# bioinformatics-centre/BayesTyper

Hardware: AMD Instinct MI355X
Metric: variant-cluster Gibbs iterations/sec + k-mer matches/sec at 1/2/4/8 MI355X (higher is better)
Workload: dtype f64 log-probabilities over u8 k-mer counts (Gibbs); u64/u8 integer (k-mer matching)

## Files before the change

bayestyper_amd/csrc/bt_gibbs_kernel.hpp:

```cpp
#pragma once
#include "bt_gibbs_tile.hpp"
#include "bt_noise_chain.hpp"
#include "bt_noise_help.hpp"
#include "bt_gibbs_simple.hpp"

namespace bt {

enum GibbsOp { OP_RUN = 0, OP_INIT_CHAIN = 1, OP_SWEEP = 2, OP_NOISE = 3, OP_RESET = 4, OP_SETUP = 5, OP_NOISE_CHAIN = 6 };

struct TraceCfg {
    uint32_t max_sweeps;
    uint32_t *counter;
    uint32_t *buf;
};

__device__ BT_NOINLINE void group_init_chain(Env env, uint32_t chain, uint32_t nvert, uint32_t nsrc, uint32_t gindex) {
    const Tile t = make_tile(env);
    const GParams BT_CAS &P = env_params(env);
    const uint32_t gseed = P.noise_seeding ? P.seed + (gindex + 1u) * (chain + 1u) : P.seed + (gindex + 1u);
    for (uint32_t v = 0; v < nvert; ++v) {
        const Vx c = make_vx(t, v);
        Env ev = env;
        const bool swap = env.resident == 0xFFFFFFFFu && t.d->hot_bytes != 0;
        if (swap) {
            hot_swap(env, v, true);
            ev.resident = v;
        }
        PROF_DECL;
        if (!make_vx(make_tile(ev), v).sc()[SC_CONSTRUCTED]) genotyper_construct(ev, v, gseed + c.cid());
        genotyper_reset(ev, v);
        if (swap) hot_swap(env, v, false);
    }
    if (nvert == 1 && nsrc == 1) return;
    uint32_t *bst = (uint32_t *)(t.base + t.d->off[A_BRNG]) + (size_t)t.plane * MT_PAD;
    mt_seed(bst, P.seed + (gindex + 1u) * (chain + 1u));
    Mt brng = mt_open(bst);
    rng_shuffle_u32(brng, t.arr<uint32_t>(A_SOURCES), nsrc);
    for (uint32_t v = 0; v < nvert; ++v) {
        const Vx c = make_vx(t, v);
        rng_shuffle_u32(brng, c.edges(), vx_ne(c));
    }
}

__device__ BT_NOINLINE void prepare_nested(Env env, uint32_t v_parent, uint32_t v_child) {
    if (env.resident != RESIDENT_ALL && env.resident != RESIDENT_NEVER) env.resident = 0xFFFFFFFFu;
    const Tile t = make_tile(env);
    const GParams BT_CAS &P = env_params(env);
    const Vx c = make_vx(t, v_parent), cc = make_vx(t, v_child);
    const uint32_t nd_n = vx_nd(c), cc_cid = cc.cid();
    const TileDesc BT_CAS &d = c.d();
    TPtr<uint32_t> ndcl = c.a<uint32_t>(A_NDCL, d.NDm > 1 ? d.NDm : 1), ndvo = c.a<uint32_t>(A_NDVOFF, d.NDm + 1);
    TPtr<uint16_t> ndv = c.a<uint16_t>(A_NDVAR, d.NDVm > 1 ? d.NDVm : 1);
    TPtr<uint32_t> pver = c.nver(), cver = cc.nver();
    for (uint32_t s = 0; s < P.S; ++s) {
        const uint32_t pv = pver[s];
        if (cver[P.S + s] == pv) continue;
        cver[P.S + s] = pv;
        cver[s] += 1;
        uint8_t ploidy = c.nest_ploidy()[s];
        uint32_t n = c.nest_n()[s];
        for (uint32_t j = 0; j < n; ++j)
            for (int q = 0; q < 4; ++q) cc.nest_stats(s, j)[q] = (double)c.nest_stats(s, j)[q];
        for (uint32_t which = 0; which < 2; ++which) {
            const uint16_t h = c.dip()[2 * s + which];
            if (h == NOHAP) continue;
            bool found = false;
            uint32_t lo = c.hn_off(h), hi = c.hn_off(h + 1);
            while (lo < hi) {
                const uint32_t mid = (lo + hi) >> 1;
                const uint32_t val = c.hn_idx(mid);
                if (val == cc_cid) {
                    found = true;
                    break;
                }
                if (val < cc_cid) lo = mid + 1;
                else hi = mid;
            }
            if (found) continue;
            ploidy = ploidy == 2 ? 1 : 0;
            uint32_t variant_idx = 0xFFFFFFFFu;
            for (uint32_t dd = 0; dd < nd_n; ++dd) {
                if (ndcl[dd] != cc_cid) continue;
                for (uint32_t i = ndvo[dd], i1 = ndvo[dd + 1]; i < i1; ++i) {
                    const uint32_t nv = ndv[i];
                    const uint32_t a = c.hap_allele(h, nv);
                    if (!is_missing(c, nv, a)) {
                        variant_idx = nv;
                        break;
                    }
                }
                break;
            }
            if (variant_idx != 0xFFFFFFFFu && n < 2) {
                for (int q = 0; q < 4; ++q) cc.nest_stats(s, n)[q] = (double)c.ksc(s, which, variant_idx)[q];
                ++n;
            }
        }
        cc.nest_ploidy()[s] = ploidy;
        cc.nest_n()[s] = (uint8_t)n;
    }
}

__device__ __forceinline__ void visit_vertex(const Env &env_in, const Tile &t, const GParams BT_CAS &P, uint32_t v, bool collect, TPtr<uint32_t> trace_row, bool tracing) {
    Env env = env_in;
    const bool swap = env.resident == 0xFFFFFFFFu && t.d->hot_bytes != 0;
    PROF_DECL;
    if (swap) {
        hot_swap(env, v, true);
        env.resident = v;
    }
    PROF(13);
    rng_topup(env, v);
    PROF(11);
    sample_diplotypes(env, v, collect, trace_row.off + v * P.S * LANES, tracing, (uint32_t *)trace_row.base);
    sample_haplotype_frequencies(env, v);
    PROF_DECL2;
    if (swap) hot_swap(env, v, false);
    PROF(13);
}

__device__ __forceinline__ void group_sweep(const Env &env, const Tile &t, const GParams BT_CAS &P, bool collect, uint32_t nvert, uint32_t nsrc, TPtr<uint32_t> trace_row, bool tracing) {
    if (tracing)
        for (uint32_t i = 0; i < t.d->nvm * P.S; ++i) trace_row[i] = 0xFFFFFFFFu;
    TPtr<uint32_t> sources = t.arr<uint32_t>(A_SOURCES), stack = t.arr<uint32_t>(A_STACK);
    TPtr<uint8_t> gploidy = t.arr<uint8_t>(A_PLOIDY);
    for (uint32_t si = 0; si < nsrc; ++si) {
        const uint32_t sv = sources[si];
        {
            const Vx root = make_vx(t, sv);
            for (uint32_t s = 0; s < P.S; ++s) {
                root.nest_ploidy()[s] = gploidy[s];
                root.nest_n()[s] = 0;
            }
        }
        uint32_t next = sv, sp = 0;
        bool have = true;
        while (have) {
            visit_vertex(env, t, P, next, collect, trace_row, tracing);
            if (nvert == 1) break;
            stack[2 * sp] = next;
            stack[2 * sp + 1] = 0;
            ++sp;
            have = false;
            while (sp > 0 && !have) {
                const uint32_t v = stack[2 * (sp - 1)];
                const uint32_t i = stack[2 * (sp - 1) + 1];
                const Vx c = make_vx(t, v);
                if (i < vx_ne(c)) {
                    stack[2 * (sp - 1) + 1] = i + 1;
                    const uint32_t tv = c.edges()[i];
                    {
                        PROF_DECL;
                        prepare_nested(env, v, tv);
                        PROF(14);
                    }
                    next = tv;
                    have = true;
                } else
                    --sp;
            }
        }
    }
}

__device__ BT_NOINLINE void noise_tally_group(Env env, uint32_t nvert, const NoiseChainCtl *nc) {
    if (env.resident != RESIDENT_ALL && env.resident != RESIDENT_NEVER) env.resident = 0xFFFFFFFFu;
    const Tile t = make_tile(env);
    const GParams BT_CAS &P = env_params(env);
    auto *bins = nc_bins(nc);
    for (uint32_t v = 0; v < nvert; ++v) {
        const Vx c = make_vx(t, v);
        const uint32_t nsu = c.sc()[SC_NSUB_U], Hm = t.d->Hm;
        const Vx::RPtr<uint8_t> sm = c.subm();
        TPtr<uint8_t> scn = c.subcnt(), sic = c.subic();
        for (uint32_t s = 0; s < P.S; ++s) {
            const uint16_t h1 = c.dip()[2 * s], h2 = c.dip()[2 * s + 1];
            const uint8_t gender = P.gender[s];
            for (uint32_t i = t.part; i < nsu; i += t.copies) {
                uint8_t m = sic[2 * i + gender];
                if (h1 != NOHAP) m = (uint8_t)(m + sm[i * Hm + h1]);
                if (h2 != NOHAP) m = (uint8_t)(m + sm[i * Hm + h2]);
                if (m == 0) nc_tally(nc, bins, s, scn[i * P.S + s]);
            }
        }
        if (t.part == 0) cache_clear(c, P, false, false);
        if (nc->help_units && help_table(t.d->cache_mode, t.d->simple, t.d->cache_entries, t.d->hoff[A_UCACHE], t.d->Dcm)) {
            if (t.copies > 1u) copies_sync();
            noise_help_publish(t, c);
        }
    }
    if (t.copies > 1u) copies_sync();
    if (nc->help_units && help_table(t.d->cache_mode, t.d->simple, t.d->cache_entries, t.d->hoff[A_UCACHE], t.d->Dcm)) __builtin_amdgcn_fence(__ATOMIC_RELEASE, "agent");
}

struct TraceRow {
    TPtr<uint32_t> row;
    bool on;
};
__device__ inline TraceRow trace_row_for(const Tile &t, const GParams BT_CAS &P, const TraceCfg &tr, uint32_t tile) {
    TraceRow r{TPtr<uint32_t>{(uint32_t BT_GAS *)tr.buf, 0u, 6u}, false};
    if (!tr.max_sweeps) return r;
    uint32_t *cnt = &tr.counter[(size_t)tile * LANES + t.lane];
    const uint32_t n = *cnt;
    if (n >= tr.max_sweeps) return r;
    *cnt = n + 1;
    r.row = TPtr<uint32_t>{(uint32_t BT_GAS *)tr.buf, (uint32_t)(t.d->trace_base + (size_t)n * t.d->nvm * P.S * LANES) + t.lane, 6u};
    r.on = true;
    return r;
}

#ifndef GIBBS_WAVES
#define GIBBS_WAVES 1
#endif
template <bool SIMPLE_ONLY>
__device__ __forceinline__ void gibbs_body(const TileDesc *__restrict__ tiles, uint8_t *__restrict__ pool, const GParams *__restrict__ Pg, int op, uint32_t arg0, uint32_t arg1,
                                           unsigned long long *__restrict__ hist, TraceCfg tr, const uint32_t *__restrict__ tile_list) {
    const uint32_t tile = kPacked ? ((const uint32_t BT_CAS *)tile_list)[2u * pack_slot()] : (tile_list ? tile_list[blockIdx.x] : blockIdx.x);
    if (kPacked && tile == 0xFFFFFFFFu) return;
    Env env{tiles, pool, Pg, tile_list, 0xFFFFFFFFu};
    const GParams BT_CAS &P = *(const GParams BT_CAS *)Pg;
    Tile t;
    t.d = (const TileDesc BT_CAS *)&tiles[tile];
    t.base = (uint8_t BT_GAS *)(pool + t.d->base);
    if (!tile_thread_active(tile_split(t.d), t.d->copies)) return;
    t.lane = tile_lane(tile_split(t.d), t.d->copies);
    t.plane = t.lane + t.d->pool_lane0;
    t.wsh = t.d->wsh;
    t.part = tile_part(t.d->copies);
    t.copies = t.d->copies;
    if (t.part != 0 && !(op == OP_RUN || op == OP_SWEEP || op == OP_INIT_CHAIN || op == OP_NOISE || op == OP_NOISE_CHAIN)) return;
    t.hot = nullptr;
    t.lds0 = kPacked ? ((const uint32_t BT_CAS *)tile_list)[2u * pack_slot() + 1u] : 0u;
    t.resident = 0xFFFFFFFFu;
    if (t.d->prio) __builtin_amdgcn_s_setprio(3);
    TPtr<uint32_t> gd = t.arr<uint32_t>(A_GDIMS);
    if (!gd[3]) return;
    const uint32_t nvert = kSingle ? 1u : (uint32_t)gd[0], nsrc = kSingle ? 1u : (uint32_t)gd[1], gindex = gd[2];
#ifdef BT_NO_NOISE_CHAIN
    const bool is_nc = false;
#else
    const bool is_nc = op == OP_NOISE_CHAIN;
#endif
    const NoiseChainCtl *nc = is_nc ? (const NoiseChainCtl *)hist : nullptr;
    const bool no_lds = is_nc && (t.d->lds_all ? t.d->hot_bytes * t.d->nvm : t.d->hot_bytes) > nc->lds_cap;
    if (no_lds) env.resident = t.resident = RESIDENT_NEVER;
    const bool whole = !no_lds && (t.d->nvm == 1 || t.d->lds_all) && t.d->hot_bytes != 0 && (op == OP_RUN || op == OP_SWEEP || op == OP_INIT_CHAIN || is_nc);
    if (whole) {
        env.resident = RESIDENT_ALL;
        for (uint32_t v = 0; v < nvert; ++v) hot_swap(env, v, true);
        t.resident = RESIDENT_ALL;
        t.hot = lds_block() + t.lds0;
    }
    const bool simple = SIMPLE_ONLY;
    if (op == OP_RUN || op == OP_SWEEP || is_nc) {
        const bool is_run = op == OP_RUN;
        const uint32_t nchains = is_run ? P.num_chains : 1u;
        uint32_t n_burn = is_run ? P.burn_in : (arg1 != 0 ? 0u : arg0), n_collect = is_run ? P.num_iterations : (arg1 != 0 ? arg0 : 0u);
        if (is_nc) {
            n_burn = nc->first_collect < nc->n_iterations ? nc->first_collect : nc->n_iterations;
            n_collect = nc->n_iterations - n_burn;
            if (!nc_begin(nc)) n_burn = n_collect = 0;
        }
        for (uint32_t chain = 0; chain < nchains; ++chain) {
            if (is_run) {
                PROF_DECL;
                group_init_chain(env, chain, nvert, nsrc, gindex);
                PROF(15);
            }
            if constexpr (SIMPLE_ONLY) {
                simple_sweeps(env, t, P, n_burn, n_collect, tr.counter, tr.buf, tr.max_sweeps, tile, nc);
                if (is_run || n_collect) drain_collected(env);
            } else {
                const uint32_t i0 = is_nc ? nc->it_begin : 0u;
                for (uint32_t i = i0; i < n_burn + n_collect; ++i) {
                    if (is_nc && i > i0) {
                        nc_phase(nc, 0x10000000u | i);
                        if (!nc_wait_table(nc, i)) break;
                        if (nc->help_units) {
                            noise_help(env, nc);
                            if (!noise_help_wait(nc, tile, i)) break;
                        }
                    }
                    if (is_nc) nc_phase(nc, 0x40000000u | i);
                    const TraceRow r = trace_row_for(t, P, tr, tile);
                    if constexpr (kSingle) {
                        if (r.on)
                            for (uint32_t q = 0; q < P.S; ++q) r.row[q] = 0xFFFFFFFFu;
                        const Vx root = make_vx(t, 0);
                        TPtr<uint8_t> gploidy = t.arr<uint8_t>(A_PLOIDY);
                        for (uint32_t q = 0; q < P.S; ++q) {
                            root.nest_ploidy()[q] = gploidy[q];
                            root.nest_n()[q] = 0;
                        }
                        visit_vertex(env, t, P, 0u, i >= n_burn, r.row, r.on);
                    } else
                        group_sweep(env, t, P, i >= n_burn, nvert, nsrc, r.row, r.on);
                    if (is_nc) {
                        nc_phase(nc, 0x50000000u | i);
                        noise_tally_group(env, nvert, nc);
                        nc_phase(nc, 0x60000000u | i);
                        if (!nc_iteration_end(nc, i)) break;
                    }
                }
                if (is_run && t.d->logged) drain_collected(env);
            }
        }
        if (!simple && (is_run || n_collect))
            for (uint32_t v = 0; v < nvert; ++v) flush_vertex(env, v);
    } else if (op == OP_INIT_CHAIN) {
        group_init_chain(env, arg0, nvert, nsrc, gindex);
        if (!SIMPLE_ONLY && arg1 != 0 && wide_table(*t.d))
            for (uint32_t v = 0; v < nvert; ++v) make_vx(t, v).sc()[SC_UC_DIRTY] = 0;
    } else if (SIMPLE_ONLY) {
    } else if (op == OP_NOISE) {
        for (uint32_t v = 0; v < nvert; ++v) {
            const Vx c = make_vx(t, v);
            const uint32_t nsu = c.sc()[SC_NSUB_U];
            TPtr<uint32_t> usub = c.usub();
            for (uint32_t s = 0; s < P.S; ++s) {
                const uint16_t h1 = c.dip()[2 * s], h2 = c.dip()[2 * s + 1];
                for (uint32_t i = t.part; i < nsu; i += t.copies) {
                    const uint32_t k = usub[i];
                    if (unique_mult(c, k, h1, h2, P.gender[s]) == 0) {
                        const uint32_t cnt = c.has_counts(k) ? c.count(k, s) : 0;
                        atomicAdd(&hist[s * 256u + cnt], 1ULL);
                    }
                }
            }
            if (t.part == 0) cache_clear(c, P, false, arg0 != 0);
        }
    } else if (op == OP_RESET) {
        for (uint32_t v = 0; v < nvert; ++v) make_vx(t, v).sc()[SC_CONSTRUCTED] = 0;
    } else if (op == OP_SETUP) {
        TPtr<uint32_t> s0 = t.arr<uint32_t>(A_SOURCES0), s1 = t.arr<uint32_t>(A_SOURCES);
        for (uint32_t i = 0; i < nsrc; ++i) s1[i] = s0[i];
        for (uint32_t v = 0; v < nvert; ++v) {
            const Vx c = make_vx(t, v);
            TPtr<uint32_t> e0 = c.a<uint32_t>(A_EDGES0, t.d->NEm > 1 ? t.d->NEm : 1), e1 = c.edges();
            for (uint32_t i = 0, n = vx_ne(c); i < n; ++i) e1[i] = e0[i];
            TPtr<uint32_t> dm = t.arr<uint32_t>(A_VDIMS, v * 8);
            SPtrF<uint32_t, LANES> sc = c.sc();
            sc[SC_H] = dm[0];
            sc[SC_V] = dm[1];
            sc[SC_NM] = dm[4];
        }
    }
    if (whole)
        for (uint32_t v = 0; v < nvert; ++v) hot_swap(env, v, false);
}
}
```

bayestyper_amd/csrc/bt_gibbs_tile.hpp:

```cpp
#pragma once
#include "bt_rng_device.hpp"

namespace bt {

constexpr unsigned LANES = 64;
constexpr uint16_t NOHAP = 0xFFFF;
constexpr double BT_LN2 = 0.693147180559945309417232121458176568;
constexpr double BT_DBL_EPS = 2.220446049250313080847263336181640625e-16;
#ifndef BT_LINEAR_DRAW_MIN
#define BT_LINEAR_DRAW_MIN 4u
#endif
#ifndef BT_UC_INVALIDATE_MIN
#define BT_UC_INVALIDATE_MIN 64u
#endif
#ifndef BT_EVAL_BLOCK
#define BT_EVAL_BLOCK 4u
#endif
constexpr uint32_t EVB = BT_EVAL_BLOCK;
#ifdef BT_SINGLE
constexpr bool kSingle = true;
#else
constexpr bool kSingle = false;
#endif
#ifdef BT_PACKED
// ... 1196 lines not shown
                v2[b] = val;
                en2[b] = st[b] == 0 || cnt != 0.0;
            }
            bool nested_any = false;
            for (uint32_t j = 0; j < 2u; ++j) nested_any = nested_any || (j < nn && (st[b] == 0 || ncnt[j] != 0.0));
            use2[b] = en2[b] && !(en1[b] && c2[b] == c1[b]);
            use3[b] = live[b] && nested_any && !(en1[b] && cn[b] == c1[b]) && !(use2[b] && cn[b] == c2[b]);
            k1[b] = k2[b] = k3[b] = KS{0, 0, 0, 0};
            if (en1[b]) k1[b] = ks_load(c.astats_cell(s, c1[b]) + 4u * st[b]);
            if (use2[b]) k2[b] = ks_load(c.astats_cell(s, c2[b]) + 4u * st[b]);
            if (use3[b]) k3[b] = ks_load(c.astats_cell(s, cn[b]) + 4u * st[b]);
        }
#pragma unroll
        for (uint32_t b = 0; b < NB; ++b) {
            if (!live[b]) continue;
            double L1[4] = {0, 0, 0, 0}, L2[4] = {0, 0, 0, 0}, L3[4] = {0, 0, 0, 0};
            uint32_t n1 = 0, n2 = 0, n3 = 0;
            if (en1[b]) L1[n1++] = v1[b];
            if (en2[b]) {
                if (use2[b]) L2[n2++] = v2[b];
                else L1[n1++] = v2[b];
            }
            for (uint32_t j = 0; j < 2u; ++j) {
                if (!(j < nn && (st[b] == 0 || ncnt[j] != 0.0))) continue;
                const double val = st[b] == 0 ? ncnt[j] : (st[b] == 1 ? nf[j] : nm[j]);
                if (en1[b] && cn[b] == c1[b]) L1[n1++] = val;
                else if (use2[b] && cn[b] == c2[b]) L2[n2++] = val;
                else L3[n3++] = val;
            }
            ks_list_rep(k1[b], L1, n1, r);
            ks_list_rep(k2[b], L2, n2, r);
            ks_list_rep(k3[b], L3, n3, r);
        }
#pragma unroll
        for (uint32_t b = 0; b < NB; ++b) {
            if (!live[b]) continue;
            if (en1[b]) ks_store(c.astats_cell(s, c1[b]) + 4u * st[b], k1[b]);
            if (use2[b]) ks_store(c.astats_cell(s, c2[b]) + 4u * st[b], k2[b]);
            if (use3[b]) ks_store(c.astats_cell(s, cn[b]) + 4u * st[b], k3[b]);
        }
    }
    dip_table_add(c, P, h1, h2, s, r);
    if (c.t.copies > 1u) copies_sync();
}

__device__ inline void flush_sample(const Vx &c, const GParams BT_CAS &P, uint32_t s) {
    const uint32_t r = c.pend()[s];
    if (r == 0) return;
    c.pend()[s] = 0;
    replay_collected(c, P, s, c.pend_dip()[2 * s], c.pend_dip()[2 * s + 1], r, (uint32_t)(double)c.pend_nest(s)[3]);
}



__device__ inline void rebuild_kmer_stats_cache(const Vx &c, const GParams BT_CAS &P, uint32_t s, uint16_t h1, uint16_t h2, uint32_t nsub_u, uint32_t nsub_m) {
    {
    const uint32_t Hm = c.d().Hm, HWm = c.d().HWm, V = c.V;
    const bool two = h2 != NOHAP;
    const uint8_t g = P.gender[s];
    const uint32_t dkey = (uint32_t)h1 | ((uint32_t)h2 << 16);
    TPtr<uint32_t> kk = c.ksc_key(s);
    uint32_t hit_way = KSC_WAYS, victim = 0;
    {
        uint32_t keys[KSC_WAYS];
#pragma unroll
        for (uint32_t e = 0; e < KSC_WAYS; ++e) keys[e] = kk[e];
        victim = kk[KSC_WAYS];
#pragma unroll
        for (uint32_t e = 0; e < KSC_WAYS; ++e)
            if (hit_way == KSC_WAYS && keys[e] == dkey) hit_way = e;
    }
    const Vx::RPtr<uint8_t> sm = c.subm();
    TPtr<uint8_t> scn = c.subcnt(), sic = c.subic();
    TPtr<uint32_t> so = c.skv_off(), sb = c.skv_bits(), msub = c.msub();
    TPtr<uint16_t> sv = c.skv_var();
    for (uint32_t a = c.t.part; a < 2 * V; a += c.t.copies) {
        const uint32_t which = a / V, var = a - which * V;
        KS acc{0, 0, 0, 0};
        const uint16_t h = which ? h2 : h1;
        if (h1 != NOHAP && (which == 0 || two)) {
            const uint32_t hw = h >> 5, hb = h & 31u;
            if (hit_way < KSC_WAYS)
                acc = ks_load(c.ksc_data(s, hit_way) + (which * c.d().Vm + var) * 4u);
            else {
            for (uint32_t i0 = 0; i0 < nsub_u; i0 += 8) {
                const uint32_t nb = nsub_u - i0 < 8u ? nsub_u - i0 : 8u;
                uint32_t eo[9];
                uint8_t dm[8], icn[8], cn[8];
#pragma unroll
                for (uint32_t q = 0; q < 9; ++q) eo[q] = q <= nb ? (uint32_t)so[i0 + q] : 0u;
#pragma unroll
                for (uint32_t q = 0; q < 8; ++q) {
                    const uint32_t i = q < nb ? i0 + q : i0;
                    uint8_t m = sm[i * Hm + h1];
                    if (two) m = (uint8_t)(m + sm[i * Hm + h2]);
                    dm[q] = q < nb ? m : (uint8_t)0;
                    icn[q] = sic[2 * i + g];
                    cn[q] = scn[i * P.S + s];
                }
                uint32_t v0[8], b0[8];
#pragma unroll
                for (uint32_t q = 0; q < 8; ++q) {
                    const bool has = q < nb && eo[q + 1] > eo[q];
                    v0[q] = has ? (uint32_t)sv[eo[q]] : 0xFFFFFFFFu;
                    b0[q] = has ? (uint32_t)sb[eo[q] * HWm + hw] : 0u;
                }
#pragma unroll
                for (uint32_t q = 0; q < 8; ++q) {
                    if (q >= nb || dm[q] == 0) continue;
                    bool hit = v0[q] == var && ((b0[q] >> hb) & 1u);
                    for (uint32_t e = eo[q] + 1; e < eo[q + 1]; ++e)
                        if (sv[e] == var && ((sb[e * HWm + hw] >> hb) & 1u)) hit = true;
                    if (hit) ks_add_r(acc, cn[q] / (double)(uint8_t)(dm[q] + icn[q]));
                }
            }
            }
        }
        if (hit_way == KSC_WAYS) ks_store(c.ksc_data(s, victim) + (which * c.d().Vm + var) * 4u, acc);
        if (h1 != NOHAP && (which == 0 || two)) {
            for (uint32_t i = 0; i < nsub_m; ++i) {
                const uint32_t k = msub[i];
                if (dip_mult(c, k, h1, h2) == 0) continue;
                bool hit = false;
                for (uint32_t e = c.kv_off(k), e1 = c.kv_off(k + 1); e < e1; ++e)
                    if (c.kv_var(e) == var && c.kv_bit(e, h)) hit = true;
                if (!hit) continue;
                const uint8_t mult = multi_mult(c, P, k, h1, h2, h1, h2, s);
                double kmer_count = 0;
                if (c.has_counts(k)) kmer_count = c.count(k, s) / (double)mult;
                ks_add_r(acc, kmer_count);
            }
        }
        ks_store(c.ksc(s, which, var), acc);
    }
    if (hit_way == KSC_WAYS) {
        kk[victim] = dkey;
        kk[KSC_WAYS] = victim + 1u < KSC_WAYS ? victim + 1u : 0u;
    }
    if (c.t.copies > 1u) copies_sync();
    }
}

__device__ inline void collect_sample_body(const Vx &c, const GParams BT_CAS &P, uint32_t s, uint32_t nsub_u, uint32_t nsub_m) {
    SPtrF<uint16_t, LANES> dip = c.dip(), pdip = c.pend_dip();
    SPtrF<uint8_t, LANES> upd = c.ksc_upd(), pvalid = c.pend_valid();
    const uint16_t h1 = dip[2 * s], h2 = dip[2 * s + 1];
    const uint8_t u = upd[s];
    const uint32_t nn = c.nest_n()[s];
    PROF_DECL;
    PROF_CNT(19, 1);
    flush_sample(c, P, s);
    PROF(16);
    {
        if (u) {
            PROF_CNT(20, 1);
            upd[s] = 0;
            c.nver()[s] += 1;
            rebuild_kmer_stats_cache(c, P, s, h1, h2, nsub_u, nsub_m);
            PROF(17);
        }
        {
            TPtr<double> pn = c.pend_nest(s);
            double nv[6] = {0, 0, 0, 0, 0, 0};
            for (uint32_t j = 0; j < 2u; ++j)
                if (j < nn) {
                    TPtr<double> q = c.nest_stats(s, j);
                    nv[3 * j] = q[0];
                    nv[3 * j + 1] = q[1];
                    nv[3 * j + 2] = q[2];
                }
            for (uint32_t j = 0; j < 2u; ++j) {
                pn[4 * j] = nv[3 * j];
                pn[4 * j + 1] = nv[3 * j + 1];
                pn[4 * j + 2] = nv[3 * j + 2];
            }
            pn[3] = (double)nn;
        }
        replay_collected(c, P, s, h1, h2, 1, nn);
        pvalid[s] = 1;
        pdip[2 * s] = h1;
        pdip[2 * s + 1] = h2;
        PROF(18);
    }
}
__device__ inline void apply_collected_log(const Vx &c, const GParams BT_CAS &P, uint32_t s, uint32_t nsub_u) {
    TPtr<uint32_t> lg = c.evlog(s);
    const uint32_t n = c.evn()[s];
    for (uint32_t e = 0; e < n; ++e) {
        const uint32_t key = lg[1 + 2 * e], r = lg[2 + 2 * e];
        const uint16_t h1 = (uint16_t)(key & 0xFFFFu), h2 = (uint16_t)(key >> 16);
        rebuild_kmer_stats_cache(c, P, s, h1, h2, nsub_u, 0);
        replay_collected(c, P, s, h1, h2, r, 0);
    }
    c.evn()[s] = 0;
}
template <bool ROOM_CHECKED = false>
__device__ inline void log_collected_run(const Vx &c, const GParams BT_CAS &P, uint32_t s, uint32_t key, uint32_t r, uint32_t nsub_u) {
    TPtr<uint32_t> lg = c.evlog(s);
    uint32_t n = c.evn()[s];
    if (!ROOM_CHECKED && n == EV_CAP) {
        apply_collected_log(c, P, s, nsub_u);
        n = 0;
    }
    lg[1 + 2 * n] = key;
    lg[2 + 2 * n] = r;
    c.evn()[s] = (uint8_t)(n + 1);
}
__device__ BT_NOINLINE void apply_full_log(Env env, uint32_t s) {
    const Vx c = make_vx(make_tile(env), 0);
    apply_collected_log(c, env_params(env), s, c.sc()[SC_NSUB_U]);
}
__device__ BT_NOINLINE void drain_collected(Env env) {
    const Vx c = make_vx(make_tile(env), 0);
    const GParams BT_CAS &P = env_params(env);
    const uint32_t nsub_u = c.sc()[SC_NSUB_U];
    SPtrF<uint16_t, LANES> pdip = c.pend_dip();
    SPtrF<uint8_t, LANES> pvalid = c.pend_valid(), upd = c.ksc_upd();
    SPtrF<uint32_t, LANES> pend = c.pend();
    for (uint32_t s = 0; s < P.S; ++s) {
        if (pvalid[s] && pend[s]) log_collected_run(c, P, s, (uint32_t)pdip[2 * s] | ((uint32_t)pdip[2 * s + 1] << 16), pend[s], nsub_u);
        pend[s] = 0;
        pvalid[s] = 0;
        upd[s] = 1;
        apply_collected_log(c, P, s, nsub_u);
    }
}

__device__ BT_NOINLINE void flush_vertex(Env env, uint32_t vtx) {
    const Vx c = make_vx(make_tile(env), vtx);
    const GParams BT_CAS &P = env_params(env);
    if (c.d().logged) {
        drain_collected(env);
        return;
    }
    for (uint32_t s = 0; s < P.S; ++s) flush_sample(c, P, s);
}
__device__ BT_NOINLINE void collect_sample_slow(Env env, uint32_t vtx, uint32_t s) {
    const Vx c = make_vx(make_tile(env), vtx);
    const GParams BT_CAS &P = env_params(env);
    SPtrF<uint32_t, LANES> sc = c.sc();
    collect_sample_body(c, P, s, sc[SC_NSUB_U], sc[SC_NSUB_M]);
}

__device__ BT_SWEEPFN void update_allele_kmer_stats(Env env, uint32_t vtx, uint32_t nsub_u, uint32_t nsub_m) {
    const Vx c = make_vx(make_tile(env), vtx);
    const GParams BT_CAS &P = env_params(env);
    SPtrF<uint16_t, LANES> dip = c.dip(), pdip = c.pend_dip();
    SPtrF<uint8_t, LANES> upd = c.ksc_upd(), pvalid = c.pend_valid();
    if (kSingle || c.d().logged) {
        SPtrF<uint32_t, LANES> pend = c.pend();
        for (uint32_t s = 0; s < P.S; ++s) {
            const uint16_t h1 = dip[2 * s], h2 = dip[2 * s + 1];
            if (pvalid[s] && pdip[2 * s] == h1 && pdip[2 * s + 1] == h2) {
                pend[s] += 1;
                continue;
            }
            if (pvalid[s] && pend[s]) {
                if (kSingle) {
                    if (c.evn()[s] == EV_CAP) apply_full_log(env, s);
                    log_collected_run<true>(c, P, s, (uint32_t)pdip[2 * s] | ((uint32_t)pdip[2 * s + 1] << 16), pend[s], nsub_u);
                } else
                    log_collected_run(c, P, s, (uint32_t)pdip[2 * s] | ((uint32_t)pdip[2 * s + 1] << 16), pend[s], nsub_u);
            }
            pdip[2 * s] = h1;
            pdip[2 * s + 1] = h2;
            pend[s] = 1;
            pvalid[s] = 1;
        }
        return;
    }
    for (uint32_t s = 0; s < P.S; ++s) {
        const uint16_t h1 = dip[2 * s], h2 = dip[2 * s + 1];
#ifndef ABL_NODEFER
#ifdef BT_NODEFER_NARROW
        if (c.t.copies == 1u)
#endif
        if (pvalid[s] && !upd[s] && pdip[2 * s] == h1 && pdip[2 * s + 1] == h2) {
            const uint32_t nn = c.nest_n()[s];
            bool same = true;
            if (nn) {
                TPtr<double> pn = c.pend_nest(s);
                same = (double)pn[3] == (double)nn;
                for (uint32_t j = 0; j < 2u; ++j)
                    if (j < nn) {
                        TPtr<double> q = c.nest_stats(s, j);
                        same = same && (double)q[0] == (double)pn[4 * j] && (double)q[1] == (double)pn[4 * j + 1] && (double)q[2] == (double)pn[4 * j + 2];
                    }
            } else
                same = true;
            if (same) {
                c.pend()[s] += 1;
                continue;
            }
        }
#endif
#ifdef BT_COLLECT_OUTLINE
        collect_sample_slow(env, vtx, s);
#else
        collect_sample_body(c, P, s, nsub_u, nsub_m);
#endif
    }
}

__device__ BT_SWEEPFN void sample_diplotypes(Env env, uint32_t vtx, bool collect, uint32_t trace_word, bool tracing, uint32_t *trace_buf) {
    const Vx c = make_vx(make_tile(env), vtx);
    const GParams BT_CAS &P = env_params(env);
    const TPtr<uint32_t> trace_row{(uint32_t BT_GAS *)uniform_ptr(trace_buf), trace_word, 6u};
    SPtrF<uint32_t, LANES> sc = c.sc();
    const uint32_t nsub_u = sc[SC_NSUB_U], nsub_m = kSingle ? 0u : (uint32_t)sc[SC_NSUB_M];
    const bool use_multi = !kSingle && sc[SC_USE_MULTI] != 0, is_sparse = sc[SC_IS_SPARSE] != 0;
    uint32_t hap_count = sc[SC_HAP_COUNT];
    PROF_DECL;
    if (sc[SC_UC_DIRTY] == 2u) {
        const Vx::UCPtr ucl = c.ucache();
        const double nan = __builtin_nan("");
        for (uint32_t i = c.t.part, n = c.d().cache_entries; i < n; i += c.t.copies) ucl[i] = nan;
        if (c.t.copies > 1u) copies_sync();
        sc[SC_UC_DIRTY] = 0;
    } else if (sc[SC_UC_DIRTY]) {
        fill_unique_cache(env, vtx);
        sc[SC_UC_DIRTY] = 0;
    }
    PROF(12);
    MtRing rng = c.rng(0);
    SPtrF<uint16_t, LANES> nzl = c.nzlist();
    SPtrF<double, LANES> logf = c.logf();
    SPtrF<uint16_t, LANES> dip = c.dip();
    uint32_t nnz = 0;
    {
        SPtrF<uint8_t, LANES> nz = c.nz();
        for (uint32_t h = 0; h < c.H; ++h)
            if (nz[h]) nzl[nnz++] = (uint16_t)h;
    }
    PROF(0);
    const uint32_t T = c.t.copies > 1u && c.d().teams > 1u ? c.d().teams : 1u;
    const uint32_t tsz = c.t.copies / T, team = c.t.part / tsz, tpart = c.t.part - team * tsz;
    const uint32_t cw = 64u / c.t.copies, gl = (threadIdx.x & 63u) % cw, tlane0 = gl + team * tsz * cw;
    SPtrF<double, LANES> cum = c.cum() + (team < T ? team : 0u) * (c.d().D2m > 1 ? c.d().D2m : 1);
    for (uint32_t s0 = 0; s0 < P.S; s0 += T) {
      double u01 = 0;
      for (uint32_t j = 0; j < T && s0 + j < P.S; ++j) {
          const double u = rng_canonical(rng);
          if (j == team) u01 = u;
      }
      PROF(24);
      const uint32_t s = s0 + team;
      uint32_t mine = 0xFFFFFFFFu;
      if (team < T && s < P.S) {
        const uint16_t p1 = dip[2 * s], p2 = dip[2 * s + 1];
        const uint8_t ploidy = c.nest_ploidy()[s];
        uint32_t gen = 0;
        if (use_multi && nsub_m) {
            multi_refresh(c, P, s, p1, p2, nsub_m);
            gen = c.mgen()[s];
        }
        PROF(1);
        const uint32_t total = ploidy == 2 ? nnz * (nnz + 1) / 2 : (ploidy == 1 ? nnz : 0u);
        const bool chain_only = total <= BT_LINEAR_DRAW_MIN;
        const bool par = !chain_only && tsz > 1u;
        double lpmax = 0;
        auto eval_candidates = [&]() {
            const bool dipl = ploidy == 2;
            const TileDesc BT_CAS &dd = c.d();
            const Vx::UCPtr uc = c.ucache();
            TPtr<double> mc = c.mcache();
            TPtr<uint32_t> uct = c.uctag(), mct = c.mctag(), mcg = c.mcgen();
            const bool multi = use_multi && nsub_m != 0;
            uint32_t a = 0, b = 0;
            auto advance = [&](uint32_t steps) {
                if (!dipl) {
                    a += steps;
                    return;
                }
                while (steps > 0 && a < nnz) {
                    const uint32_t left = nnz - b;
                    if (steps < left) {
                        b += steps;
                        steps = 0;
                    } else {
                        steps -= left;
                        ++a;
                        b = a;
                    }
                }
            };
            const uint32_t stride_blocks = par ? tsz : 1u;
            if (par) advance(EVB * tpart);
            lpmax = -__builtin_huge_val();
            for (uint32_t base = par ? EVB * tpart : 0u; base < total; base += EVB * stride_blocks) {
                const uint32_t nb = total - base < EVB ? total - base : EVB;
                uint16_t ha[EVB], hb[EVB];
                uint32_t uslot[EVB], ukey[EVB];
                double uval[EVB], mval[EVB], la[EVB], lb[EVB];
                uint32_t utag[EVB], mtag[EVB], mgn[EVB];
#pragma unroll
                for (uint32_t q = 0; q < EVB; ++q) {
                    if (q < nb) {
                        ha[q] = nzl[a];
                        hb[q] = dipl ? (uint16_t)nzl[b] : NOHAP;
                        if (dipl) {
                            if (++b == nnz) {
                                ++a;
                                b = a;
                            }
                        } else
                            ++a;
                        const uint32_t idx = dip_index(c, ha[q], hb[q]);
                        ukey[q] = s * dd.Dcm + idx + 1u;
                        uslot[q] = dd.cache_mode == 0 ? s * dd.Dcm + idx : hashed_slot(c, ukey[q]);
                        uval[q] = dd.cache_mode != 2 ? (double)uc[uslot[q]] : 0.0;
                        utag[q] = dd.cache_mode == 1 ? (uint32_t)uct[uslot[q]] : 0u;
                        if (multi) {
                            mtag[q] = mct[uslot[q]];
                            mgn[q] = mcg[uslot[q]];
                            mval[q] = mc[uslot[q]];
                        }
                        la[q] = logf[ha[q]];
                        lb[q] = dipl ? (double)logf[hb[q]] : 0.0;
                    }
                }
                if (multi) {
                    bool need[EVB], any = false;
#pragma unroll
                    for (uint32_t q = 0; q < EVB; ++q) {
                        need[q] = q < nb && !(mtag[q] == ukey[q] && mgn[q] == gen);
                        any = any || need[q];
                    }
                    if (any) {
                        double fresh[EVB];
                        multi_log_prob_block(c, P, s, ha, hb, need, nsub_m, fresh);
#pragma unroll
                        for (uint32_t q = 0; q < EVB; ++q)
                            if (need[q]) {
                                mval[q] = fresh[q];
                                mct[uslot[q]] = ukey[q];
                                mcg[uslot[q]] = gen;
                                mc[uslot[q]] = fresh[q];
                            }
                    }
                }
                {
                    bool umiss[EVB], any = false;
#pragma unroll
                    for (uint32_t q = 0; q < EVB; ++q) {
                        umiss[q] = q < nb && !((dd.cache_mode == 0 && uval[q] == uval[q]) || (dd.cache_mode == 1 && utag[q] == ukey[q]));
                        any = any || umiss[q];
                    }
                    if (any) {
                        double fresh[EVB];
                        unique_log_prob_block(c, P, s, ha, hb, umiss, nsub_u, fresh);
#pragma unroll
                        for (uint32_t q = 0; q < EVB; ++q)
                            if (umiss[q]) uval[q] = fresh[q];
                    }
                }
#pragma unroll
                for (uint32_t q = 0; q < EVB; ++q) {
                    if (q < nb) {
                        double lp = 0;
                        if (!dipl) lp += la[q];
                        else if (ha[q] == hb[q]) lp += 2 * la[q];
                        else lp += BT_LN2 + la[q] + lb[q];
                        lp += uval[q];
                        if (multi) lp += mval[q];
                        lpmax = lp > lpmax ? lp : lpmax;
                        cum[base + q] = lp;
                    }
                }
                if (par) advance(EVB * (stride_blocks - 1u));
            }
            if (par) {
                const double own = lpmax;
                for (uint32_t m = 0; m < tsz; ++m) {
                    const double o = __shfl(own, (int)(tlane0 + m * cw));
                    lpmax = o > lpmax ? o : lpmax;
                }
                copies_sync();
            }
        };
        auto chain_pick = [&](double u01) -> uint32_t {
            if (total == 0) return 0u;
            double run = cum[0];
            for (uint32_t i = 1; i < total; ++i) {
                run = log_addition((double)cum[i], run);
                cum[i] = run;
            }
            const double u = bt_log(u01) + run;
            uint32_t lo = 0, hi = total;
            while (lo < hi) {
                const uint32_t mid = (lo + hi) >> 1;
                if (u < cum[mid]) hi = mid;
                else lo = mid + 1;
            }
            return lo < total ? lo : total - 1;
        };
        uint32_t pick = 0;
        for (bool exact = chain_only;; exact = true) {
            eval_candidates();
            PROF(2);
            if (exact) {
                if (total == 0) (void)bt_log(u01);
                pick = chain_pick(u01);
                PROF(28);
                break;
            }
            double acc = 0, thr = 0, off = 0;
            uint32_t s0 = 0, s1 = total;
            {
                const uint32_t ncp = tsz, L = (total + ncp - 1u) / ncp;
                const uint32_t i0 = tpart * L < total ? tpart * L : total, i1 = i0 + L < total ? i0 + L : total;
                double run = 0;
                for (uint32_t b0 = i0; b0 < i1; b0 += 8) {
                    double e[8];
#pragma unroll
                    for (uint32_t q = 0; q < 8; ++q) e[q] = b0 + q < i1 ? (double)cum[b0 + q] : 0.0;
#pragma unroll
                    for (uint32_t q = 0; q < 8; ++q)
                        if (b0 + q < i1) e[q] = bt_exp(e[q] - lpmax);
#pragma unroll
                    for (uint32_t q = 0; q < 8; ++q)
                        if (b0 + q < i1) {
                            run += e[q];
                            cum[b0 + q] = run;
                        }
                }
                for (uint32_t m = 0; m < ncp; ++m) acc += __shfl(run, (int)(tlane0 + m * cw));
                thr = u01 * acc;
                uint32_t seg = ncp;
                for (uint32_t m = 0; m < ncp; ++m) {
                    const double tseg = __shfl(run, (int)(tlane0 + m * cw));
                    if (seg == ncp) {
                        if (thr < off + tseg) seg = m;
                        else off += tseg;
                    }
                }
                if (tsz > 1u) copies_sync();
                s0 = seg * L < total ? seg * L : total;
                s1 = s0 + L < total ? s0 + L : total;
            }
            PROF(25);
            uint32_t lo = s0, hi = s1;
            while (lo < hi) {
                const uint32_t mid = (lo + hi) >> 1;
                if (thr < off + (double)cum[mid]) hi = mid;
                else lo = mid + 1;
            }
            const double amax = fabs(lpmax) > 1.0 ? fabs(lpmax) : 1.0;
            double margin = 64.0 * (double)total * amax * BT_DBL_EPS;
            margin = (margin > 1e-6 ? margin : 1e-6) * acc;
            const bool safe = lo < s1 && off + (double)cum[lo] - thr > margin && (lo == 0 || thr - (lo == s0 ? off : off + (double)cum[lo - 1]) > margin);
            PROF(26);
            if (safe) {
                pick = lo;
                break;
            }
            PROF_CNT(14, 1000000);
        }
        uint16_t h1 = NOHAP, h2 = NOHAP;
        if (ploidy == 2) {
            uint32_t a = 0, rem = pick;
            while (rem >= nnz - a) {
                rem -= nnz - a;
                ++a;
            }
            h1 = nzl[a];
            h2 = nzl[a + rem];
        } else if (ploidy == 1) {
            h1 = nzl[pick];
        }
        mine = (uint32_t)h1 | ((uint32_t)h2 << 16);
      }
      if (T > 1u) copies_sync();
      PROF(3);
      for (uint32_t j = 0; j < T && s0 + j < P.S; ++j) {
        const uint32_t ss = s0 + j;
        const uint32_t hh = T > 1u ? (uint32_t)__shfl((int)mine, (int)(gl + j * tsz * cw)) : mine;
        const uint16_t h1 = (uint16_t)(hh & 0xFFFFu), h2 = (uint16_t)(hh >> 16);
        const uint16_t p1 = dip[2 * ss], p2 = dip[2 * ss + 1];
        dip[2 * ss] = h1;
        dip[2 * ss + 1] = h2;
        if (!kSingle && c.d().nvm > 1u && (h1 != p1 || h2 != p2)) c.nver()[ss] += 1;
        hfd_increment(c, h1, is_sparse, hap_count);
        hfd_increment(c, h2, is_sparse, hap_count);
        PROF(4);
        update_multicluster_multiplicities(c, P, h1, h2, p1, p2, ss, nsub_m);
        PROF(5);
        if (tracing) trace_row[ss] = hh;
      }
    }
    mt_close(rng);
    sc[SC_HAP_COUNT] = hap_count;
#ifndef ABL_NOSTATS
    if (collect) update_allele_kmer_stats(env, vtx, nsub_u, nsub_m);
#endif
    PROF(6);
    sc[SC_USE_MULTI] = nsub_m != 0 ? 1u : 0u;
}

__device__ BT_SWEEPFN void rng_topup(Env env, uint32_t vtx) {
    const Vx c = make_vx(make_tile(env), vtx);
    MtRing a = c.rng(0), b = c.rng(1);
    a.topup();
    b.topup();
    mt_close(a);
    mt_close(b);
}

template <typename Q>
__device__ inline uint32_t simplex_prob_vector(const Vx &c, const GParams BT_CAS &P, Q out, uint32_t total_obs, uint32_t plus_size) {
    const uint32_t Hn = c.H;
    const double BT_GAS *lg = P.lgamma_int;
    const double sparsity = c.sparsity();
    const double lsp = bt_log(sparsity), l1sp = bt_log(1 - sparsity);
    double prob_z_log = plus_size * lsp + (Hn - plus_size) * l1sp;
    double prob_t_log = lg[plus_size] - lg[total_obs + plus_size];
    double prob_eq_z_log = 0.0 + prob_z_log + prob_t_log;
    double row_sum = prob_eq_z_log;
    uint32_t n = 0;
    out[n++] = row_sum;
    double prev = row_sum;
    for (uint32_t j = plus_size + 1; j < Hn + 1; ++j) {
        const double cardinal = lg[Hn - plus_size + 1] - (lg[j - plus_size + 1] + lg[Hn - j + 1]);
        prob_z_log = j * lsp + (Hn - j) * l1sp;
        prob_t_log = lg[j] - lg[total_obs + j];
        prob_eq_z_log = cardinal + prob_z_log + prob_t_log;
        row_sum += bt_log(1 + bt_exp(prob_eq_z_log - row_sum));
        out[n++] = row_sum;
        const double a = row_sum, b = prev;
        const double mn = a < b ? a : b;
        prev = row_sum;
        if (a == b || fabs(a - b) < fabs(mn) * BT_DBL_EPS * 100) break;
    }
    for (uint32_t i = 0; i < n; ++i) out[i] = bt_exp((double)out[i] - row_sum);
    return n;
}

template <class G>
__device__ inline double rng_gamma_count(G &rng, NormalState nd, const GParams BT_CAS &P, uint32_t count) {
    const uint32_t ai = count + 1u;
    const double a1 = (double)ai - 1.0 / 3.0;
    const double a2 = ai < P.gamma_n ? (double)P.gamma_a2[ai] : 1.0 / sqrt(9.0 * a1);
    return a1 * rng_gamma_v(rng, nd, a1, a2) * 1.0;
}

__device__ BT_SWEEPFN void sample_haplotype_frequencies(Env env, uint32_t vtx) {
    const Vx c = make_vx(make_tile(env), vtx);
    const GParams BT_CAS &P = env_params(env);
    const TileDesc BT_CAS &d = c.d();
    SPtrF<uint32_t, LANES> sc = c.sc();
    const uint32_t n_obs = sc[SC_HAP_COUNT];
    PROF_DECL;
    if (n_obs > 0) {
        MtRing rng = c.rng(1);
        const NormalState nd = c.fnd();
        SPtrF<uint32_t, LANES> obs = c.obs();
        SPtrF<double, LANES> freq = c.freq();
        SPtrF<uint8_t, LANES> nz = c.nz();
        if (!sc[SC_IS_SPARSE]) {
            double norm = 0;
            for (uint32_t h = 0; h < c.H; ++h) {
                const double f = rng_gamma_count(rng, nd, P, obs[h]);
                freq[h] = f;
                norm += f;
                obs[h] = 0;
            }
            SPtrF<double, LANES> logf = c.logf();
            for (uint32_t h = 0; h < c.H; ++h) {
                const double f = freq[h] / norm;
                freq[h] = f;
                logf[h] = bt_log(f);
            }
        } else {
            Vx::HSet plus = c.plus_set(), zero = c.zero_set();
            SPtrF<uint32_t, LANES> unext = c.unext();
            const uint32_t plus_size = uset_size(plus);
            uint32_t len;
            TPtr<double> vec = c.simplex();
            const bool cached = d.scache_n && n_obs <= 2 * d.S && plus_size <= d.scache_p;
            const uint32_t ci = cached ? (n_obs - 1) * d.scache_p + (plus_size - 1) : 0u;
            if (cached) vec = c.scache() + (uint32_t)ci * d.scache_len;
            constexpr uint32_t PRE = 4;
            const uint32_t pre = d.scache_len < PRE ? d.scache_len : PRE;
            double head[PRE];
#pragma unroll
            for (uint32_t q = 0; q < PRE; ++q) head[q] = (cached && q < pre) ? (double)vec[q] : 0.0;
            len = cached ? (uint32_t)c.sclen()[ci] : 0u;
            if (len == 0) {
                len = simplex_prob_vector(c, P, vec, n_obs, plus_size);
                if (cached) c.sclen()[ci] = len;
#pragma unroll
                for (uint32_t q = 0; q < PRE; ++q) head[q] = q < len ? (double)vec[q] : 0.0;
            }
            PROF(21);
            const double u = rng_canonical(rng);
            uint32_t ub = 0;
#pragma unroll
            for (uint32_t q = 0; q < PRE; ++q)
                if (ub == q && q < len && !(u < head[q])) ub = q + 1;
            if (ub == PRE)
                while (ub < len && !(u < vec[ub])) ++ub;
            const uint32_t simplex_size = ub + plus_size;
            double norm = 0;
            for (uint32_t e = uset_begin(plus); e != US_NONE; e = unext[e]) {
                const double f = rng_gamma_count(rng, nd, P, obs[e]);
                freq[e] = f;
                norm += f;
                nz[e] = 2;
            }
            PROF(22);
            while (uset_size(plus) < simplex_size) {
                const uint32_t pos = rng_uniform_int(rng, uset_size(zero));
                uint32_t e = uset_begin(zero);
                for (uint32_t i = 0; i < pos; ++i) e = unext[e];
                const double f = rng_gamma_count(rng, nd, P, 0u);
                freq[e] = f;
                norm += f;
                nz[e] = 2;
                uset_erase(zero, e);
                uset_insert(plus, e);
            }
            PROF(23);
            {
                uint32_t h = 0;
                for (; h + 8 <= c.H; h += 8) {
                    uint8_t m8[8];
#pragma unroll
                    for (int q = 0; q < 8; ++q) m8[q] = nz[h + q];
#pragma unroll
                    for (int q = 0; q < 8; ++q) {
                        if (m8[q] == 2) nz[h + q] = 1;
                        else {
                            freq[h + q] = 0;
                            nz[h + q] = 0;
                            obs[h + q] = 0;
                        }
                    }
                }
                for (; h < c.H; ++h) {
                    if (nz[h] == 2) nz[h] = 1;
                    else {
                        freq[h] = 0;
                        nz[h] = 0;
                        obs[h] = 0;
                    }
                }
            }
            SPtrF<uint16_t, LANES> nzl = c.nzlist();
            uint32_t np = 0;
            for (uint32_t e = uset_begin(plus); e != US_NONE; e = unext[e]) nzl[np++] = (uint16_t)e;
            uset_clear(plus);
            for (uint32_t i = 0; i < np; ++i) {
                const uint32_t e = nzl[i];
                const double f = freq[e] / norm;
                freq[e] = f;
                c.logf()[e] = bt_log(f);
                uset_insert(zero, e);
                obs[e] = 0;
            }
        }
        mt_close(rng);
    }
    PROF(7);
    sc[SC_HAP_COUNT] = 0;
}

}
```

Baseline: 1.208 billion.

## Unify dense/sparse frequency sampling loop and split normalization across tile copies

Merges the dense and sparse haplotype-frequency gamma sampling into a single wave-uniform loop, so lanes on different paths advance together instead of diverging. The full-H cleanup scan of nz flags is replaced by a walk over only the previously nonzero list, whose count is now returned by sample_diplotypes. The normalization and log pass is strided across tile copies and followed by a copies sync. This reduces divergent control flow and O(H) scans, at the cost of an extra sync and more reliance on the nzlist count being correct.

```diff
diff --git a/bayestyper_amd/csrc/bt_gibbs_kernel.hpp b/bayestyper_amd/csrc/bt_gibbs_kernel.hpp
--- a/bayestyper_amd/csrc/bt_gibbs_kernel.hpp
+++ b/bayestyper_amd/csrc/bt_gibbs_kernel.hpp
@@ -112,8 +112,8 @@
     PROF(13);
     rng_topup(env, v);
     PROF(11);
-    sample_diplotypes(env, v, collect, trace_row.off + v * P.S * LANES, tracing, (uint32_t *)trace_row.base);
-    sample_haplotype_frequencies(env, v);
+    const uint32_t nnz = sample_diplotypes(env, v, collect, trace_row.off + v * P.S * LANES, tracing, (uint32_t *)trace_row.base);
+    sample_haplotype_frequencies(env, v, nnz);
     PROF_DECL2;
     if (swap) hot_swap(env, v, false);
     PROF(13);
diff --git a/bayestyper_amd/csrc/bt_gibbs_tile.hpp b/bayestyper_amd/csrc/bt_gibbs_tile.hpp
--- a/bayestyper_amd/csrc/bt_gibbs_tile.hpp
+++ b/bayestyper_amd/csrc/bt_gibbs_tile.hpp
@@ -1522,7 +1522,7 @@
     }
 }
 
-__device__ BT_SWEEPFN void sample_diplotypes(Env env, uint32_t vtx, bool collect, uint32_t trace_word, bool tracing, uint32_t *trace_buf) {
+__device__ BT_SWEEPFN uint32_t sample_diplotypes(Env env, uint32_t vtx, bool collect, uint32_t trace_word, bool tracing, uint32_t *trace_buf) {
     const Vx c = make_vx(make_tile(env), vtx);
     const GParams BT_CAS &P = env_params(env);
     const TPtr<uint32_t> trace_row{(uint32_t BT_GAS *)uniform_ptr(trace_buf), trace_word, 6u};
@@ -1815,6 +1815,7 @@
 #endif
     PROF(6);
     sc[SC_USE_MULTI] = nsub_m != 0 ? 1u : 0u;
+    return nnz;
 }
 
 __device__ BT_SWEEPFN void rng_topup(Env env, uint32_t vtx) {
@@ -1863,7 +1864,7 @@
     return a1 * rng_gamma_v(rng, nd, a1, a2) * 1.0;
 }
 
-__device__ BT_SWEEPFN void sample_haplotype_frequencies(Env env, uint32_t vtx) {
+__device__ BT_SWEEPFN void sample_haplotype_frequencies(Env env, uint32_t vtx, uint32_t nnz) {
     const Vx c = make_vx(make_tile(env), vtx);
     const GParams BT_CAS &P = env_params(env);
     const TileDesc BT_CAS &d = c.d();
@@ -1876,23 +1877,11 @@
         SPtrF<uint32_t, LANES> obs = c.obs();
         SPtrF<double, LANES> freq = c.freq();
         SPtrF<uint8_t, LANES> nz = c.nz();
-        if (!sc[SC_IS_SPARSE]) {
-            double norm = 0;
-            for (uint32_t h = 0; h < c.H; ++h) {
-                const double f = rng_gamma_count(rng, nd, P, obs[h]);
-                freq[h] = f;
-                norm += f;
-                obs[h] = 0;
-            }
-            SPtrF<double, LANES> logf = c.logf();
-            for (uint32_t h = 0; h < c.H; ++h) {
-                const double f = freq[h] / norm;
-                freq[h] = f;
-                logf[h] = bt_log(f);
-            }
-        } else {
-            Vx::HSet plus = c.plus_set(), zero = c.zero_set();
-            SPtrF<uint32_t, LANES> unext = c.unext();
+        const bool is_sparse = sc[SC_IS_SPARSE] != 0;
+        Vx::HSet plus = c.plus_set(), zero = c.zero_set();
+        SPtrF<uint32_t, LANES> unext = c.unext();
+        uint32_t n_first = c.H, n_steps = c.H, cur = 0;
+        if (is_sparse) {
             const uint32_t plus_size = uset_size(plus);
             uint32_t len;
             TPtr<double> vec = c.simplex();
@@ -1919,65 +1908,77 @@
                 if (ub == q && q < len && !(u < head[q])) ub = q + 1;
             if (ub == PRE)
                 while (ub < len && !(u < vec[ub])) ++ub;
-            const uint32_t simplex_size = ub + plus_size;
-            double norm = 0;
-            for (uint32_t e = uset_begin(plus); e != US_NONE; e = unext[e]) {
-                const double f = rng_gamma_count(rng, nd, P, obs[e]);
+            n_first = plus_size;
+            n_steps = ub + plus_size;
+            cur = uset_begin(plus);
+        }
+        double norm = 0;
+        for (uint32_t i = 0; bt_wave_any(i < n_steps); ++i) {
+            if (i < n_steps) {
+                uint32_t e, o = 0;
+                const bool adding = i >= n_first;
+                if (!is_sparse) e = i;
+                else if (!adding) {
+                    e = cur;
+                    cur = unext[e];
+                } else {
+                    const uint32_t pos = rng_uniform_int(rng, uset_size(zero));
+                    e = uset_begin(zero);
+                    for (uint32_t q = 0; q < pos; ++q) e = unext[e];
+                }
+                if (!adding) o = obs[e];
+                const double f = rng_gamma_count(rng, nd, P, o);
                 freq[e] = f;
                 norm += f;
-                nz[e] = 2;
-            }
-            PROF(22);
-            while (uset_size(plus) < simplex_size) {
-                const uint32_t pos = rng_uniform_int(rng, uset_size(zero));
-                uint32_t e = uset_begin(zero);
-                for (uint32_t i = 0; i < pos; ++i) e = unext[e];
-                const double f = rng_gamma_count(rng, nd, P, 0u);
-                freq[e] = f;
-                norm += f;
-                nz[e] = 2;
-                uset_erase(zero, e);
-                uset_insert(plus, e);
-            }
-            PROF(23);
-            {
-                uint32_t h = 0;
-                for (; h + 8 <= c.H; h += 8) {
-                    uint8_t m8[8];
-#pragma unroll
-                    for (int q = 0; q < 8; ++q) m8[q] = nz[h + q];
-#pragma unroll
-                    for (int q = 0; q < 8; ++q) {
-                        if (m8[q] == 2) nz[h + q] = 1;
-                        else {
-                            freq[h + q] = 0;
-                            nz[h + q] = 0;
-                            obs[h + q] = 0;
-                        }
+                if (!is_sparse) obs[e] = 0;
+                else {
+                    nz[e] = 2;
+                    if (adding) {
+                        uset_erase(zero, e);
+                        uset_insert(plus, e);
+                        PROF(23);
+                    } else {
+                        PROF(22);
                     }
                 }
-                for (; h < c.H; ++h) {
-                    if (nz[h] == 2) nz[h] = 1;
-                    else {
-                        freq[h] = 0;
-                        nz[h] = 0;
-                        obs[h] = 0;
-                    }
+            }
+        }
+        PROF(23);
+        const uint32_t part = c.t.part, copies = c.t.copies;
+        SPtrF<double, LANES> logf = c.logf();
+        if (!is_sparse) {
+            for (uint32_t h = part; h < c.H; h += copies) {
+                const double f = freq[h] / norm;
+                freq[h] = f;
+                logf[h] = bt_log(f);
+            }
+        } else {
+            SPtrF<uint16_t, LANES> nzl = c.nzlist();
+            for (uint32_t i = 0; i < nnz; ++i) {
+                const uint32_t h = nzl[i];
+                if (nz[h] != 2) {
+                    freq[h] = 0;
+                    nz[h] = 0;
+                    obs[h] = 0;
                 }
             }
-            SPtrF<uint16_t, LANES> nzl = c.nzlist();
             uint32_t np = 0;
             for (uint32_t e = uset_begin(plus); e != US_NONE; e = unext[e]) nzl[np++] = (uint16_t)e;
             uset_clear(plus);
-            for (uint32_t i = 0; i < np; ++i) {
+            for (uint32_t i = part; i < np; i += copies) {
                 const uint32_t e = nzl[i];
                 const double f = freq[e] / norm;
                 freq[e] = f;
-                c.logf()[e] = bt_log(f);
+                logf[e] = bt_log(f);
+            }
+            for (uint32_t i = 0; i < np; ++i) {
+                const uint32_t e = nzl[i];
+                nz[e] = 1;
                 uset_insert(zero, e);
                 obs[e] = 0;
             }
         }
+        if (copies > 1u) copies_sync();
         mt_close(rng);
     }
     PROF(7);
```

New measurement: 1.225 billion (median of 6 runs). +1.3%, better.
